# citibeth/spsparse

Measured on AMD Instinct MI355X. Metric: nnz(C)/s for C=A*A SpGEMM, higher is better.
Workload: dtype f64

## Files before the change

### spsparse_amd/csrc/consolidate.hip

```cpp
#include "internal.h"
#include "devutil.h"

namespace spsamd {

__global__ void k_inspect(const int32_t *major, const int32_t *minor, const double *val, size_t n,
	uint64_t nrow, uint64_t ncol, int zero_nan, uint32_t *flags)
{
	uint32_t f = 0;
	for (size_t i = (size_t)blockIdx.x * blockDim.x + threadIdx.x; i < n; i += (size_t)gridDim.x * blockDim.x) {
		int32_t r = major[i], c = minor[i];
		if (r < 0 || (uint64_t)r >= nrow || c < 0 || (uint64_t)c >= ncol) f |= 1u;
		double v = val[i];
		if (v == 0 || (zero_nan && v != v)) f |= 2u | 8u;
		if (i > 0) {
			int32_t pr = major[i - 1], pc = minor[i - 1];
			if (!(pr < r || (pr == r && pc < c))) f |= 2u;
			if (pr > r) f |= 16u;
			if (pr > r || (pr == r && pc > c)) f |= 32u;
			if (!(pc < c || (pc == c && pr < r))) f |= 4u;
		}
	}
	__shared__ uint32_t s_f;
	if (threadIdx.x == 0) s_f = 0;
	__syncthreads();
	uint32_t wf = 0;
#pragma unroll
	for (uint32_t b = 1u; b <= 32u; b <<= 1) if (__ballot(f & b)) wf |= b;
	if (wf && lane_id() == 0) atomicOr(&s_f, wf);
	__syncthreads();
	if (threadIdx.x == 0 && s_f && (*(volatile uint32_t *)flags & s_f) != s_f) atomicOr(flags, s_f);
}

__device__ __forceinline__ uint64_t ref_key(uint64_t key, int minor_bits, int major_bits, int swap)
{
	if (!swap) return key;
	const uint64_t minor = key & ((uint64_t(1) << minor_bits) - 1), major = key >> minor_bits;
	return (minor << major_bits) | major;
}

__global__ void k_gather_flag(const double *val, const uint32_t *perm, const uint64_t *keys, size_t n, int zero_nan,
	int minor_bits, int major_bits, int swap, double *sval, uint8_t *keep, unsigned long long *first_key)
{
	size_t i = (size_t)blockIdx.x * blockDim.x + threadIdx.x;
	if (i >= n) return;
	double v = val[perm[i]];
	sval[i] = v;
	keep[i] = (v != 0) ? 1 : 0;
	if (zero_nan && v != 0 && v == v) atomicMin(first_key, (unsigned long long)ref_key(keys[i], minor_bits, major_bits, swap));
}

__global__ void k_first_pos(const double *sval, const uint32_t *perm, const uint64_t *keys, size_t n,
	int minor_bits, int major_bits, int swap, const unsigned long long *first_key, uint32_t *first_pos)
{
	size_t i = (size_t)blockIdx.x * blockDim.x + threadIdx.x;
	if (i >= n) return;
	const double v = sval[i];
	if (v != 0 && v == v && ref_key(keys[i], minor_bits, major_bits, swap) == *first_key) atomicMin(first_pos, perm[i]);
}

__global__ void k_apply_first(const double *sval, const uint32_t *perm, const uint64_t *keys, uint8_t *keep, size_t n,
	int minor_bits, int major_bits, int swap, const unsigned long long *first_key, const uint32_t *first_pos)
{
	size_t i = (size_t)blockIdx.x * blockDim.x + threadIdx.x;
	if (i >= n) return;
	const double v = sval[i];
	if (v == v) return;
	const uint64_t k = ref_key(keys[i], minor_bits, major_bits, swap), fk = *first_key;
	if (k < fk || (k == fk && perm[i] < *first_pos)) keep[i] = 0;
}

__global__ void k_compact(const uint64_t *keys, const double *sval, const uint8_t *keep, const uint32_t *pos, size_t n,
	uint64_t *kk, double *kv)
{
	size_t i = (size_t)blockIdx.x * blockDim.x + threadIdx.x;
	if (i < n && keep[i]) {
		uint32_t p = pos[i];
		kk[p] = keys[i];
		kv[p] = sval[i];
	}
}

__global__ void k_heads(const uint64_t *kk, const uint32_t *nk_ptr, size_t n, uint8_t *head)
{
	size_t j = (size_t)blockIdx.x * blockDim.x + threadIdx.x;
	if (j >= n) return;
	uint32_t nk = *nk_ptr;
	head[j] = (j < nk && (j == 0 || kk[j] != kk[j - 1])) ? 1 : 0;
}

__global__ void k_merge(const uint64_t *kk, const double *kv, const uint8_t *head, const uint32_t *hpos,
	const uint32_t *nk_ptr, size_t n, int minor_bits, int policy,
	int32_t *row, int32_t *col, double *val)
{
	size_t j = (size_t)blockIdx.x * blockDim.x + threadIdx.x;
	if (j >= n || !head[j]) return;
	uint32_t nk = *nk_ptr;
	uint64_t key = kk[j];
	double acc = kv[j];
	for (size_t t = j + 1; t < nk && kk[t] == key; ++t) {
		if (policy == SPSAMD_ADD) acc += kv[t];
		else if (policy == SPSAMD_REPLACE) acc = kv[t];
	}
	uint32_t o = hpos[j];
	row[o] = (int32_t)(key >> minor_bits);
	col[o] = (int32_t)(key & ((uint64_t(1) << minor_bits) - 1));
	val[o] = acc;
}

__global__ void k_min_key(unsigned long long *first_key, const unsigned long long *global_key)
{
	if (*global_key < *first_key) *first_key = *global_key;
}

uint32_t inspect_operand(spsamd_ctx *c, const int32_t *major, const int32_t *minor, const double *val, size_t n,
	uint64_t nrow, uint64_t ncol)
{
	uint32_t *flags = c->arena.get<uint32_t>(1);
	fill_zero(c, flags, sizeof(uint32_t));
	if (n) {
		k_inspect<<<dim3(std::min(grid_for(n, 1024), 2048u)), dim3(256), 0, c->stream>>>(major, minor, val, n, nrow, ncol, 0, flags);
		SPS_LAUNCH_CHECK();
	}
	return read_back(c, flags);
}

void consolidate_operand(spsamd_ctx *c, const spsamd_coo *X, int lead, int ref_lead, int duplicate_policy, int zero_nan, ConMat *out,
	Prepared **prep, const unsigned long long *global_first_key)
{
	if (prep) *prep = nullptr;
// ... 21 lines not shown
	const int32_t *d1 = to_device(c, X->idx1, n, X->mem);
	const double *dv = to_device(c, X->val, n, X->mem);
	const int32_t *major = lead == 0 ? d0 : d1;
	const int32_t *minor = lead == 0 ? d1 : d0;

	uint32_t *flags = c->arena.get<uint32_t>(2);
	fill_zero(c, flags, 2 * sizeof(uint32_t));
	k_inspect<<<dim3(std::min(grid_for(n, 1024), 2048u)), dim3(256), 0, c->stream>>>(major, minor, dv, n, out->nrow, out->ncol, zero_nan, flags);
	SPS_LAUNCH_CHECK();
	uint32_t f = read_back(c, flags);
	if (f & 1u) throw Error{SPSAMD_EINVAL, "Sparse index out of bounds (VectorCooArray::add would reject it, VectorCooArray.hpp:246-262)"};

	if (X->sort0 == lead && (f & 16u))
		throw Error{SPSAMD_EINVAL, "operand claims sort_order but its leading index is not ascending (set_sorted() on unsorted tuples?)"};
	if ((X->sort0 == lead && !(zero_nan && ref_lead != lead && (f & 2u))) || !(f & 2u)) {
		out->row = const_cast<int32_t *>(major);
		out->col = const_cast<int32_t *>(minor);
		out->val = const_cast<double *>(dv);
		out->nnz = (uint32_t)n;
		return;
	}

	int mb = bits_of(out->ncol), Mb = bits_of(out->nrow);
	PairSort sort(c, n);
	build_keys(c, major, minor, n, mb, sort.keys);
	const int low_bit = (f & 4u) ? 0 : mb;
	sort.run(mb + Mb, low_bit);
	uint64_t *ks = sort.keys;
	uint32_t *ps = sort.perm;
	uint64_t *kk = sort.spare_keys;
	if (!(f & 4u) && !(f & 8u)) {
		out->row = c->arena.get<int32_t>(n);
		out->col = c->arena.get<int32_t>(n);
		out->val = c->arena.get<double>(n);
		gather_sorted(c, ks, ps, dv, n, mb, out->row, out->col, out->val);
		out->nnz = (uint32_t)n;
		return;
	}

	double *sval = c->arena.get<double>(n);
	uint8_t *keep = c->arena.get<uint8_t>(n);
	unsigned long long *first_key = c->arena.get<unsigned long long>(1);
	uint32_t *first_pos = flags + 1;
	const int swap = ref_lead != lead ? 1 : 0;
	if (zero_nan) {
		SPS_HIP(hipMemsetAsync(first_key, 0xFF, sizeof(unsigned long long), c->stream));
		fill_u32(c, first_pos, 0xFFFFFFFFu, 1);
	}
	k_gather_flag<<<dim3(grid_for(n)), dim3(256), 0, c->stream>>>(dv, ps, ks, n, zero_nan, mb, Mb, swap, sval, keep, first_key);
	SPS_LAUNCH_CHECK();
	if (zero_nan) {
		if (global_first_key) { k_min_key<<<dim3(1), dim3(1), 0, c->stream>>>(first_key, global_first_key); SPS_LAUNCH_CHECK(); }
		k_first_pos<<<dim3(grid_for(n)), dim3(256), 0, c->stream>>>(sval, ps, ks, n, mb, Mb, swap, first_key, first_pos);
		SPS_LAUNCH_CHECK();
		k_apply_first<<<dim3(grid_for(n)), dim3(256), 0, c->stream>>>(sval, ps, ks, keep, n, mb, Mb, swap, first_key, first_pos);
		SPS_LAUNCH_CHECK();
	}
	uint32_t *pos = c->arena.get<uint32_t>(n + 1);
	scan_exclusive_u8_u32(c, keep, pos, n);
	double *kv = c->arena.get<double>(n);
	k_compact<<<dim3(grid_for(n)), dim3(256), 0, c->stream>>>(ks, sval, keep, pos, n, kk, kv);
	SPS_LAUNCH_CHECK();
	uint8_t *head = keep;
	k_heads<<<dim3(grid_for(n)), dim3(256), 0, c->stream>>>(kk, pos + n, n, head);
	SPS_LAUNCH_CHECK();
	uint32_t *hpos = c->arena.get<uint32_t>(n + 1);
	scan_exclusive_u8_u32(c, head, hpos, n);
	out->row = c->arena.get<int32_t>(n);
	out->col = c->arena.get<int32_t>(n);
	out->val = c->arena.get<double>(n);
	k_merge<<<dim3(grid_for(n)), dim3(256), 0, c->stream>>>(kk, kv, head, hpos, pos + n, n, mb, duplicate_policy,
		out->row, out->col, out->val);
	SPS_LAUNCH_CHECK();
	out->nnz = read_back(c, hpos + n);
}

__global__ void k_first_key_raw(const int32_t *major, const int32_t *minor, const double *val, size_t n, int minor_bits, int major_bits, int swap,
	unsigned long long *first_key)
{
	unsigned long long best = ~0ull;
	for (size_t i = (size_t)blockIdx.x * blockDim.x + threadIdx.x; i < n; i += (size_t)gridDim.x * blockDim.x) {
		const double v = val[i];
		if (v != 0 && v == v) {
			const uint64_t key = ((uint64_t)(uint32_t)major[i] << minor_bits) | (uint64_t)(uint32_t)minor[i];
			const unsigned long long k = ref_key(key, minor_bits, major_bits, swap);
			best = k < best ? k : best;
		}
	}
#pragma unroll
	for (int d = 32; d >= 1; d >>= 1) { const unsigned long long o = __shfl_xor(best, d, 64); best = o < best ? o : best; }
	if (lane_id() == 0 && best != ~0ull) atomicMin(first_key, best);
}

void first_kept_key_raw(spsamd_ctx *c, const spsamd_coo *Xdev, int lead, int ref_lead, unsigned long long *out_dev)
{
	SPS_HIP(hipMemsetAsync(out_dev, 0xFF, sizeof(unsigned long long), c->stream));
	const size_t n = Xdev->nnz;
	if (!n) return;
	const uint64_t shape[2] = {Xdev->shape0, Xdev->shape1};
	const int mb = bits_of(shape[1 - lead]), Mb = bits_of(shape[lead]);
	const int32_t *major = lead == 0 ? Xdev->idx0 : Xdev->idx1, *minor = lead == 0 ? Xdev->idx1 : Xdev->idx0;
	k_first_key_raw<<<dim3(std::min(grid_for(n), 2048u)), dim3(256), 0, c->stream>>>(major, minor, Xdev->val, n, mb, Mb, ref_lead != lead ? 1 : 0, out_dev);
	SPS_LAUNCH_CHECK();
}

uint32_t *sorted_permutation(spsamd_ctx *c, const spsamd_coo *X, int lead)
{
	size_t n = X->nnz;
	if (n >= (size_t(1) << 31)) throw Error{SPSAMD_EINVAL, "operand has 2^31 or more tuples"};
	if (n == 0) return nullptr;
	if (!X->idx0 || !X->idx1) throw Error{SPSAMD_EINVAL, "operand with nnz > 0 has a null array"};
	uint64_t shape[2] = {X->shape0, X->shape1};
	const int32_t *d0 = to_device(c, X->idx0, n, X->mem);
	const int32_t *d1 = to_device(c, X->idx1, n, X->mem);
	const int32_t *major = lead == 0 ? d0 : d1;
	const int32_t *minor = lead == 0 ? d1 : d0;
	int mb = bits_of(shape[1 - lead]), Mb = bits_of(shape[lead]);
	PairSort sort(c, n);
	build_keys(c, major, minor, n, mb, sort.keys);
	sort.run(mb + Mb);
	return sort.perm;
}


__global__ void k_row_flags(const int32_t *row, size_t n, uint8_t *flag)
{
	size_t i = (size_t)blockIdx.x * blockDim.x + threadIdx.x;
	if (i < n) flag[i] = (i == 0 || row[i] != row[i - 1]) ? 1 : 0;
}

__global__ void k_row_starts(const int32_t *row, const uint8_t *flag, const uint32_t *pos, size_t n, uint32_t *beg, int32_t *id)
{
	size_t i = (size_t)blockIdx.x * blockDim.x + threadIdx.x;
	if (i >= n) return;
	if (flag[i]) {
		beg[pos[i]] = (uint32_t)i;
		id[pos[i]] = row[i];
	}
	if (i == n - 1) beg[pos[n]] = (uint32_t)n;
}

void dim_beginnings(spsamd_ctx *c, const ConMat &m, RowList *out)
{
	size_t n = m.nnz;
	out->nrows = 0;
	out->beg = c->arena.get<uint32_t>(n + 1);
	out->id = c->arena.get<int32_t>(n ? n : 1);
	if (n == 0) return;
	uint8_t *flag = c->arena.get<uint8_t>(n);
	uint32_t *pos = c->arena.get<uint32_t>(n + 1);
	k_row_flags<<<dim3(grid_for(n)), dim3(256), 0, c->stream>>>(m.row, n, flag);
	SPS_LAUNCH_CHECK();
	scan_exclusive_u8_u32(c, flag, pos, n);
	k_row_starts<<<dim3(grid_for(n)), dim3(256), 0, c->stream>>>(m.row, flag, pos, n, out->beg, out->id);
	SPS_LAUNCH_CHECK();
	out->nrows = read_back(c, pos + n);
}


__global__ void k_rowptr(const int32_t *row, uint32_t n, uint64_t nptr, uint32_t *ptr)
{
	uint64_t r = (uint64_t)blockIdx.x * blockDim.x + threadIdx.x;
	if (r >= nptr) return;
	uint32_t lo = 0, hi = n;
	while (lo < hi) {
		uint32_t mid = lo + ((hi - lo) >> 1);
		if ((uint64_t)(uint32_t)row[mid] < r) lo = mid + 1; else hi = mid;
	}
	ptr[r] = lo;
}

__global__ void k_rowptr_scatter(const int32_t *row, uint32_t n, uint64_t nptr, uint32_t *ptr)
{
	const uint64_t t = (uint64_t)blockIdx.x * blockDim.x + threadIdx.x;
	uint64_t first = 0, last = 0;
	if (t > 0 && t < n) {
		first = (uint64_t)(uint32_t)row[t - 1] + 1;
		last = std::min<uint64_t>((uint64_t)(uint32_t)row[t] + 1, nptr);
	}
// ... 69 lines not shown
```

### spsparse_amd/csrc/internal.h

```cpp
#pragma once

#include <hip/hip_runtime.h>
#include <stdint.h>
#include <stddef.h>
#include <string>
#include <vector>

#include "../../include/spsparse_amd.h"

namespace spsamd {


struct Error {
	int code;
	std::string msg;
};

#define SPS_HIP(call)                                                              \
	do {                                                                           \
		hipError_t e_ = (call);                                                    \
		if (e_ != hipSuccess)                                                      \
			throw ::spsamd::Error{SPSAMD_EHIP, std::string(#call) + ": " + hipGetErrorString(e_)}; \
	} while (0)

// ... 117 lines not shown
	EV_N3 = 6,
	EV_END = 7,
	EV_N4 = 8,
	EV_FETCH0 = EV_N4, EV_FETCH1 = 9 };
enum Ev2 { EV2_TILES_BEGIN = 0, EV2_TILES_END = 1, EV2_DIRECT_END = 2 };


void scan_exclusive_u32_i64(spsamd_ctx *c, const uint32_t *in, int64_t *out, size_t n);
void scan_exclusive_u32_u32(spsamd_ctx *c, const uint32_t *in, uint32_t *out, size_t n);
void scan_exclusive_u8_u32(spsamd_ctx *c, const uint8_t *in, uint32_t *out, size_t n);
void scan_exclusive_u64_u64(spsamd_ctx *c, const unsigned long long *in, unsigned long long *out, size_t n);

constexpr int SCAN_BATCH_MAX = 12;
struct ScanBatch { const uint32_t *in[SCAN_BATCH_MAX]; uint32_t *out[SCAN_BATCH_MAX]; int count = 0;
	void add(const uint32_t *i, uint32_t *o) { in[count] = i; out[count] = o; ++count; } };
void scan_exclusive_u32_batch(spsamd_ctx *c, const ScanBatch &b, size_t n);

constexpr int WORD_LIST_MAX = 40;
struct WordList { const uint32_t *p[WORD_LIST_MAX]; int count = 0;
	int add(const void *q) { p[count] = (const uint32_t *)q; return count++; }
	int add64(const void *q) { const int at = add(q); add((const uint32_t *)q + 1); return at; } };
void read_back_words(spsamd_ctx *c, const WordList &w, uint32_t *host);

struct PairSort {
	uint64_t *keys;
	uint32_t *perm;
	uint64_t *spare_keys;
	uint32_t *spare_pay;
	PairSort(spsamd_ctx *c, size_t n);
	void run(int key_bits, int low_bit = 0);
private:
	spsamd_ctx *c;
	size_t n;
};

void fill_u32(spsamd_ctx *c, uint32_t *p, uint32_t v, size_t n);
void fill_zero(spsamd_ctx *c, void *p, size_t bytes);
template <class T> T *get_zeroed(spsamd_ctx *c, size_t n) { T *p = c->arena.get<T>(n); fill_zero(c, p, n * sizeof(T)); return p; }

template <class T>
T read_back(spsamd_ctx *c, const T *dev)
{
	T *h = (T *)c->host_staging(sizeof(T));
	SPS_HIP(hipMemcpyAsync(h, dev, sizeof(T), hipMemcpyDeviceToHost, c->stream));
	SPS_HIP(hipStreamSynchronize(c->stream));
	return *h;
}

inline unsigned grid_for(size_t n, unsigned bs = 256) { return (unsigned)((n + bs - 1) / bs); }

#define SPSAMD_MEM_DEVICE_VERIFIED 3


struct Prepared;
// ... 14 lines not shown
	if (mem != SPSAMD_MEM_HOST || n == 0) return p;
	T *d = c->arena.get<T>(n);
	SPS_HIP(hipMemcpyAsync(d, p, n * sizeof(T), hipMemcpyHostToDevice, c->stream));
	return d;
}

struct PlainStream {
	const int32_t *major = nullptr, *minor = nullptr;
	const double *val = nullptr;
	uint32_t flags = 0;
	bool own_result = false;
};
PlainStream plain_stream(spsamd_ctx *c, const spsamd_coo &X, int lead);

struct MaskKeys {
	const int32_t *i = nullptr, *j = nullptr;
	uint32_t n = 0;
	Prepared *prep = nullptr;
};
void mask_keys(spsamd_ctx *c, const spsamd_coo *M, int lead, uint64_t nrow, uint64_t ncol, MaskKeys *out);

int bits_of(uint64_t dim);
void build_keys(spsamd_ctx *c, const int32_t *major, const int32_t *minor, size_t n, int minor_bits, uint64_t *keys);
void gather_sorted(spsamd_ctx *c, const uint64_t *keys, const uint32_t *perm, const double *val, size_t n, int minor_bits,
	int32_t *row, int32_t *col, double *oval);

struct ProductFrame {
	int a0, a1, bk, bj;
	uint64_t nrow, inner, ncol;
	uint64_t inner_b;
	uint64_t shape0, shape1;
	ProductFrame(const spsamd_coo *A, char transpose_A, const spsamd_coo *B, char transpose_B, bool permute);
	void check_inner(const char *what) const;
};
bool product_is_empty(double C, const spsamd_vec *scalei, const spsamd_coo *A, const spsamd_vec *scalej, const spsamd_coo *B,
	const spsamd_vec *scalek);


struct ConMat {
	int32_t *row = nullptr;
	int32_t *col = nullptr;
	double *val = nullptr;
	uint32_t nnz = 0;
	uint64_t nrow = 0, ncol = 0;
};


void consolidate_operand(spsamd_ctx *c, const spsamd_coo *X, int lead, int ref_lead, int duplicate_policy,
	int zero_nan, ConMat *out, Prepared **prep = nullptr, const unsigned long long *global_first_key = nullptr);

void first_kept_key_raw(spsamd_ctx *c, const spsamd_coo *Xdev, int lead, int ref_lead, unsigned long long *out_dev);

uint32_t inspect_operand(spsamd_ctx *c, const int32_t *major, const int32_t *minor, const double *val, size_t n,
	uint64_t nrow, uint64_t ncol);

struct RowList {
	uint32_t *beg = nullptr;
	int32_t *id = nullptr;
	uint32_t nrows = 0;
};
void dim_beginnings(spsamd_ctx *c, const ConMat &m, RowList *out);

uint32_t *sorted_permutation(spsamd_ctx *c, const spsamd_coo *X, int lead);

uint32_t *dense_rowptr(spsamd_ctx *c, const ConMat &m, uint32_t extra, uint32_t *into = nullptr);

struct __attribute__((packed, aligned(4))) BTup { int32_t col; uint32_t vlo, vhi; };

struct SolveSchedule {
	bool built = false;
	uint32_t levels = 0, max_level_rows = 0;
	uint64_t tuples_used = 0;
	int64_t zero_pivot = -1;
	uint32_t *level_ptr = nullptr;
	uint32_t *rows = nullptr;
	std::vector<uint32_t> h_level_ptr, h_level_max;
};

struct Prepared {
	spsamd_ctx *ctx = nullptr;
	ConMat m;
	int lead = 0;
	bool owns = false;
	std::vector<void *> owned;
// ... 141 lines not shown
```

### spsparse_amd/csrc/k_add.hip

```cpp
#include "internal.h"
#include "devutil.h"
#include "x86fp.h"

#include <algorithm>
#include <cstdio>
#include <cstring>

namespace spsamd {

struct FirstKept {
	unsigned long long key;
	uint32_t src, idx;
};

__device__ __forceinline__ uint64_t add_key(const int32_t *row, const int32_t *col, uint32_t i)
{
	return ((uint64_t)(uint32_t)row[i] << 32) | (uint64_t)(uint32_t)col[i];
}

__device__ __forceinline__ bool before_first(uint64_t key, uint32_t src, uint32_t idx, const FirstKept &f)
{
	return key < f.key || (key == f.key && (src < f.src || (src == f.src && idx < f.idx)));
}

// ... 161 lines not shown
}

static void add_stream(spsamd_ctx *c, const spsamd_coo *X, int lead, bool force_sort, AddStream *out, bool *sorted)
{
	*out = AddStream();
	const OperandView view = operand_view(c, X);
	if (view.prep && view.prep->lead == lead && !force_sort) { const ConMat &m = view.prep->m; out->row = m.row; out->col = m.col; out->val = m.val; out->n = m.nnz; return; }
	X = &view.coo;
	const size_t n = X->nnz;
	if (n == 0) return;
	const uint64_t shape[2] = {X->shape0, X->shape1};
	const PlainStream ps = plain_stream(c, *X, lead);
	const int32_t *major = ps.major, *minor = ps.minor;
	const double *dv = ps.val;
	const bool ordered = ps.own_result ? X->sort0 == lead : !(ps.flags & 32u);
	const int low_bit = !ps.own_result && !(ps.flags & 4u) ? -1 : 0;
	if (ordered && !force_sort) { out->row = major; out->col = minor; out->val = dv; out->n = (uint32_t)n; return; }
	const int mb = bits_of(shape[1 - lead]), Mb = bits_of(shape[lead]);
	PairSort sort(c, n);
	build_keys(c, major, minor, n, mb, sort.keys);
	sort.run(mb + Mb, low_bit < 0 ? mb : 0);
	int32_t *row = c->arena.get<int32_t>(n), *col = c->arena.get<int32_t>(n);
	double *val = c->arena.get<double>(n);
	gather_sorted(c, sort.keys, sort.perm, dv, n, mb, row, col, val);
	out->row = row; out->col = col; out->val = val; out->n = (uint32_t)n;
	*sorted = true;
}

template <int MODE>
static void launch_merge(spsamd_ctx *c, uint32_t ntiles, const AddStream &a, const AddStream &b, double alpha, double beta,
	int zero_nan, const FirstKept *first, const uint32_t *split, uint32_t *tile_count, const uint32_t *tile_off,
	int32_t *orow, int32_t *ocol, double *oval)
{
	k_add_merge<MODE><<<dim3(ntiles), dim3(ADD_NT), 0, c->stream>>>(a, b, alpha, beta, zero_nan, first, split, tile_count, tile_off, orow, ocol, oval);
	SPS_LAUNCH_CHECK();
}

void add_matrices(spsamd_ctx *c, double alpha, const spsamd_coo *A, char transpose_A, double beta, const spsamd_coo *B,
	char transpose_B, int duplicate_policy, int zero_nan, int sink_kind, int sink_flags, spsamd_result *res)
{
	check_sink_args(duplicate_policy, sink_kind);
	std::memset(res, 0, sizeof(*res));
	const int la = transpose_A == 'T' ? 1 : 0, lb = transpose_B == 'T' ? 1 : 0;
	const uint64_t ash[2] = {A->shape0, A->shape1}, bsh[2] = {B->shape0, B->shape1};
	const uint64_t nrow = ash[la], ncol = ash[1 - la];
	if (nrow != bsh[lb] || ncol != bsh[1 - lb]) {
		char buf[200];
// ... 55 lines not shown
```

### spsparse_amd/csrc/operand.hip

```cpp
#include "internal.h"
#include "devutil.h"

#include <algorithm>
#include <cstdio>

namespace spsamd {

OperandView operand_view(spsamd_ctx *c, const spsamd_coo *X)
{
	OperandView v;
	v.coo = *X;
	if (X->mem != SPSAMD_MEM_PREPARED) return v;
	Prepared *p = (Prepared *)const_cast<int32_t *>(X->idx0);
	if (!p || p->ctx != c) throw Error{SPSAMD_EINVAL, "a prepared operand belongs to the context that prepared it"};
	v.prep = p;
	v.coo.idx0 = p->lead == 0 ? p->m.row : p->m.col; v.coo.idx1 = p->lead == 0 ? p->m.col : p->m.row; v.coo.val = p->m.val;
	v.coo.nnz = p->m.nnz; v.coo.sort0 = p->lead; v.coo.mem = SPSAMD_MEM_DEVICE;
	return v;
}

uint64_t operand_tuples(const spsamd_coo *X)
{
	if (X->mem == SPSAMD_MEM_PREPARED) return X->idx0 ? ((const Prepared *)X->idx0)->m.nnz : 0;
	return X->nnz;
// ... 12 lines not shown
bool is_own_result(const spsamd_ctx *c, const spsamd_coo &X)
{
	if (X.mem != SPSAMD_MEM_DEVICE) return false;
	for (const auto &o : c->own)
		if (o.sort0 >= 0 && o.sort0 == X.sort0 && o.d0 == X.idx0 && o.d1 == X.idx1 && o.v == X.val && o.nnz == X.nnz &&
			o.shape0 == X.shape0 && o.shape1 == X.shape1) return true;
	return false;
}

int bits_of(uint64_t dim)
{
	int b = 0;
	while (b < 63 && (uint64_t(1) << b) < dim) ++b;
	return b;
}

__global__ void __launch_bounds__(256) k_build_keys(const int32_t *__restrict__ major, const int32_t *__restrict__ minor, uint32_t n,
	int minor_bits, uint64_t *__restrict__ keys)
{
	const uint32_t i = blockIdx.x * blockDim.x + threadIdx.x;
	if (i < n) keys[i] = ((uint64_t)(uint32_t)major[i] << minor_bits) | (uint64_t)(uint32_t)minor[i];
}

__global__ void __launch_bounds__(256) k_gather_sorted(const uint64_t *__restrict__ keys, const uint32_t *__restrict__ perm,
	const double *__restrict__ val, uint32_t n, int minor_bits, int32_t *__restrict__ row, int32_t *__restrict__ col,
	double *__restrict__ oval)
{
	const uint32_t i = blockIdx.x * blockDim.x + threadIdx.x;
	if (i >= n) return;
	const uint64_t k = keys[i];
	row[i] = (int32_t)(k >> minor_bits);
	col[i] = (int32_t)(k & ((uint64_t(1) << minor_bits) - 1));
	oval[i] = val[perm[i]];
}

void build_keys(spsamd_ctx *c, const int32_t *major, const int32_t *minor, size_t n, int minor_bits, uint64_t *keys)
{
	k_build_keys<<<dim3(grid_for(n)), dim3(256), 0, c->stream>>>(major, minor, (uint32_t)n, minor_bits, keys);
	SPS_LAUNCH_CHECK();
}

void gather_sorted(spsamd_ctx *c, const uint64_t *keys, const uint32_t *perm, const double *val, size_t n, int minor_bits,
	int32_t *row, int32_t *col, double *oval)
{
	k_gather_sorted<<<dim3(grid_for(n)), dim3(256), 0, c->stream>>>(keys, perm, val, (uint32_t)n, minor_bits, row, col, oval);
	SPS_LAUNCH_CHECK();
}

PlainStream plain_stream(spsamd_ctx *c, const spsamd_coo &X, int lead)
{
	check_operand(X, OPERAND_VALUES | OPERAND_PLAIN_MEM);
	const size_t n = X.nnz;
	const uint64_t shape[2] = {X.shape0, X.shape1};
	PlainStream s;
	s.own_result = is_own_result(c, X);
	const int32_t *d0 = to_device(c, X.idx0, n, X.mem), *d1 = to_device(c, X.idx1, n, X.mem);
	s.val = to_device(c, X.val, n, X.mem);
	s.major = lead == 0 ? d0 : d1; s.minor = lead == 0 ? d1 : d0;
	if (s.own_result) return s;
	s.flags = inspect_operand(c, s.major, s.minor, s.val, n, shape[lead], shape[1 - lead]);
	if (s.flags & 1u) throw Error{SPSAMD_EINVAL, "Sparse index out of bounds (VectorCooArray::add would reject it, VectorCooArray.hpp:246-262)"};
	if (X.sort0 == lead && (s.flags & 32u))
		throw Error{SPSAMD_EINVAL, "operand claims sort_order but its (row, col) keys are not in that order (set_sorted() on unsorted tuples?)"};
	return s;
}


__global__ void __launch_bounds__(256) k_mask_inspect(const int32_t *__restrict__ r, const int32_t *__restrict__ c, size_t n,
// ... 104 lines not shown
```

### spsparse_amd/csrc/prims.hip

```cpp
#include "internal.h"
#include "devutil.h"

#include <utility>

namespace spsamd {


static size_t round_up(size_t x, size_t a) { return (x + a - 1) / a * a; }

void *Arena::alloc(size_t bytes)
{
	bytes = round_up(bytes ? bytes : 1, 256);
	call_used += bytes;
	if (!slabs.empty()) {
		Slab &s = slabs.back();
		if (s.used + bytes <= s.cap) {
			void *p = s.p + s.used;
			s.used += bytes;
			return p;
		}
	}
	size_t cap = bytes > (size_t(256) << 20) ? bytes : (size_t(256) << 20);
	if (cap < high_water / 2) cap = high_water / 2;
	Slab s{nullptr, cap, 0};
// ... 302 lines not shown
{
	const int i = (int)threadIdx.x;
	if (i < w.count) dst[i] = *w.p[i];
}

void read_back_words(spsamd_ctx *c, const WordList &w, uint32_t *host)
{
	if (w.count == 0) return;
	uint32_t *dev = c->arena.get<uint32_t>(WORD_LIST_MAX);
	k_collect_words<<<dim3(1), dim3(64), 0, c->stream>>>(w, dev);
	SPS_LAUNCH_CHECK();
	uint32_t *h = (uint32_t *)c->host_staging(sizeof(uint32_t) * WORD_LIST_MAX);
	SPS_HIP(hipMemcpyAsync(h, dev, sizeof(uint32_t) * (size_t)w.count, hipMemcpyDeviceToHost, c->stream));
	SPS_HIP(hipStreamSynchronize(c->stream));
	for (int i = 0; i < w.count; ++i) host[i] = h[i];
}


constexpr int RS_NT = 256;
constexpr int RS_NW = RS_NT / 64;
constexpr int RS_ITER = 16;
constexpr int RS_TILE = RS_NT * RS_ITER;

template <int BITS>
__global__ __launch_bounds__(RS_NT) void k_rs_hist(const uint64_t *keys, size_t n, int shift, uint32_t *ghist, unsigned nblocks)
{
	constexpr int NB = 1 << BITS;
	__shared__ uint32_t hist[NB];
	for (int d = threadIdx.x; d < NB; d += RS_NT) hist[d] = 0;
	__syncthreads();
	size_t base = (size_t)blockIdx.x * RS_TILE;
#pragma unroll 4
	for (int q = 0; q < RS_ITER; ++q) {
		size_t i = base + (size_t)q * RS_NT + threadIdx.x;
		if (i < n) atomicAdd(&hist[(unsigned)(keys[i] >> shift) & (unsigned)(NB - 1)], 1u);
	}
	__syncthreads();
	for (int d = threadIdx.x; d < NB; d += RS_NT) ghist[(size_t)d * nblocks + blockIdx.x] = hist[d];
}

template <int BITS>
__global__ __launch_bounds__(RS_NT) void k_rs_scatter(const uint64_t *keys, const uint32_t *pay, size_t n, int shift,
	const uint32_t *gbase, unsigned nblocks, uint64_t *keys_out, uint32_t *pay_out, int iota_payload)
{
	constexpr int NB = 1 << BITS;
	constexpr int DPT = NB / RS_NT;
	__shared__ uint32_t wcnt[RS_NW][NB];
	__shared__ uint32_t gdelta[NB];
	__shared__ uint32_t scr[RS_NW + 1];
	__shared__ uint64_t s_key[RS_TILE];
	__shared__ uint32_t s_pay[RS_TILE];
	const unsigned w = wave_id(), lane = lane_id();
	for (int q = threadIdx.x; q < RS_NW * NB; q += RS_NT) (&wcnt[0][0])[q] = 0;
	__syncthreads();
	const size_t tile = (size_t)blockIdx.x * RS_TILE;
	const size_t wbase = tile + (size_t)w * (RS_ITER * 64);
	uint64_t key[RS_ITER];
#pragma unroll
	for (int q = 0; q < RS_ITER; ++q) {
		size_t i = wbase + (size_t)q * 64 + lane;
		key[q] = i < n ? keys[i] : 0;
		if (i < n) atomicAdd(&wcnt[w][(unsigned)(key[q] >> shift) & (unsigned)(NB - 1)], 1u);
	}
	__syncthreads();
	{
		uint32_t tot[DPT], mine = 0;
#pragma unroll
		for (int x = 0; x < DPT; ++x) {
			const unsigned d = threadIdx.x * DPT + x;
			tot[x] = 0;
#pragma unroll
			for (int ww = 0; ww < RS_NW; ++ww) tot[x] += wcnt[ww][d];
			mine += tot[x];
		}
		uint32_t lbase = block_exclusive_scan<uint32_t, RS_NT>(mine, scr, (uint32_t *)nullptr);
#pragma unroll
		for (int x = 0; x < DPT; ++x) {
			const unsigned d = threadIdx.x * DPT + x;
			gdelta[d] = gbase[(size_t)d * nblocks + blockIdx.x] - lbase;
			uint32_t run = lbase;
#pragma unroll
			for (int ww = 0; ww < RS_NW; ++ww) {
				uint32_t t = wcnt[ww][d];
				wcnt[ww][d] = run;
// ... 2 lines not shown
			lbase += tot[x];
		}
	}
	__syncthreads();
#pragma unroll
	for (int q = 0; q < RS_ITER; ++q) {
		size_t i = wbase + (size_t)q * 64 + lane;
		bool valid = i < n;
		unsigned digit = (unsigned)(key[q] >> shift) & (unsigned)(NB - 1);
		uint64_t peers = __ballot(valid);
#pragma unroll
		for (int b = 0; b < BITS; ++b) {
			bool bit = (digit >> b) & 1u;
			uint64_t m = __ballot(valid && bit);
			peers &= bit ? m : ~m;
		}
		unsigned rank = __popcll(peers & lanemask_lt());
		uint32_t old = 0;
		if (valid && rank == 0) old = atomicAdd(&wcnt[w][digit], (uint32_t)__popcll(peers));
		int leader = valid ? (__ffsll((unsigned long long)peers) - 1) : (int)lane;
		old = __shfl(old, leader, 64);
		if (valid) {
			s_key[old + rank] = key[q];
			s_pay[old + rank] = iota_payload ? (uint32_t)i : pay[i];
		}
	}
	__syncthreads();
	const uint32_t nvalid = (uint32_t)(n - tile < (size_t)RS_TILE ? n - tile : (size_t)RS_TILE);
	for (uint32_t p = threadIdx.x; p < nvalid; p += RS_NT) {
		const uint64_t k = s_key[p];
		const uint32_t dst = gdelta[(unsigned)(k >> shift) & (unsigned)(NB - 1)] + p;
		keys_out[dst] = k;
		pay_out[dst] = s_pay[p];
	}
}

template <int BITS>
static int radix_sort_pairs_bits(spsamd_ctx *c, uint64_t *keys0, uint32_t *pay0, uint64_t *keys1, uint32_t *pay1, size_t n, int key_bits, int low_bit)
{
	constexpr size_t NB = size_t(1) << BITS;
	int passes = (key_bits - low_bit + BITS - 1) / BITS;
	unsigned nblocks = (unsigned)((n + RS_TILE - 1) / RS_TILE);
	uint32_t *ghist = c->arena.get<uint32_t>(NB * nblocks);
	uint32_t *gbase = c->arena.get<uint32_t>(NB * nblocks + 1);
	uint64_t *ksrc = keys0, *kdst = keys1;
	uint32_t *psrc = pay0, *pdst = pay1;
	int where = 0;
	if (passes == 0) passes = 1;
	for (int p = 0; p < passes; ++p) {
		int shift = low_bit + BITS * p;
		k_rs_hist<BITS><<<dim3(nblocks), dim3(RS_NT), 0, c->stream>>>(ksrc, n, shift, ghist, nblocks);
		SPS_LAUNCH_CHECK();
		scan_exclusive_u32_u32(c, ghist, gbase, NB * nblocks);
		k_rs_scatter<BITS><<<dim3(nblocks), dim3(RS_NT), 0, c->stream>>>(ksrc, psrc, n, shift, gbase, nblocks, kdst, pdst, p == 0);
		SPS_LAUNCH_CHECK();
		uint64_t *tk = ksrc; ksrc = kdst; kdst = tk;
		uint32_t *tp = psrc; psrc = pdst; pdst = tp;
		where ^= 1;
	}
	return where;
}

static int radix_sort_pairs(spsamd_ctx *c, uint64_t *keys0, uint32_t *pay0, uint64_t *keys1, uint32_t *pay1, size_t n, int key_bits, int low_bit)
{
	if (n == 0) return 0;
	if (low_bit < 0 || low_bit > key_bits) low_bit = 0;
	return radix_sort_pairs_bits<8>(c, keys0, pay0, keys1, pay1, n, key_bits, low_bit);
}

PairSort::PairSort(spsamd_ctx *c, size_t n) : c(c), n(n)
{
	keys = c->arena.get<uint64_t>(n); spare_keys = c->arena.get<uint64_t>(n);
	perm = c->arena.get<uint32_t>(n); spare_pay = c->arena.get<uint32_t>(n);
}

void PairSort::run(int key_bits, int low_bit)
{
	if (radix_sort_pairs(c, keys, perm, spare_keys, spare_pay, n, key_bits, low_bit)) {
		std::swap(keys, spare_keys);
		std::swap(perm, spare_pay);
	}
}

}
```

### spsparse_amd/csrc/spgemm.hip

```cpp
#include "spgemm_host.h"

namespace spsamd {

__global__ void k_pack_b(const int32_t *bcol, const double *bval, uint32_t n, BTup *out)
{
	uint32_t i = blockIdx.x * blockDim.x + threadIdx.x;
	if (i >= n) return;
	double v = bval[i];
	BTup t; t.col = bcol[i]; t.vlo = (uint32_t)__double2loint(v); t.vhi = (uint32_t)__double2hiint(v);
	out[i] = t;
}


__global__ void k_elem_len(const int32_t *acol, const uint32_t *bptr, uint32_t n, uint32_t *lo, uint32_t *len)
{
	uint32_t e = blockIdx.x * blockDim.x + threadIdx.x;
	if (e < n) { int32_t k = acol[e]; uint32_t b = bptr[k]; lo[e] = b; len[e] = bptr[k + 1] - b; }
}

__global__ void k_apply_scalej(const int32_t *acol, const double *aval, uint32_t n, const int32_t *pos, const double *sval,
	int32_t ninner, int32_t *acol2, double *aval2)
{
	uint32_t e = blockIdx.x * blockDim.x + threadIdx.x;
	if (e >= n) return;
// ... 344 lines not shown
	Prepared *need[2]; int n = 0;
	if (!pa->have_maxlen) need[n++] = pa;
	if (pb != pa && !pb->have_maxlen) need[n++] = pb;
	if (!n) return;
	uint32_t *mx = get_zeroed<uint32_t>(c, 2);
	for (int q = 0; q < n; ++q) {
		k_max_rowlen<<<dim3(std::min(grid_for(need[q]->m.nrow, 1024), 1024u)), dim3(256), 0, st>>>(need[q]->rowptr, need[q]->m.nrow, mx + q);
		SPS_LAUNCH_CHECK();
	}
	struct { uint32_t a, b; } hm = read_back(c, (const decltype(hm) *)mx);
	need[0]->maxlen = hm.a; need[0]->have_maxlen = true;
	if (n > 1) { need[1]->maxlen = hm.b; need[1]->have_maxlen = true; }
}

void prepared_row_structure(spsamd_ctx *c, Prepared *p)
{
	ensure_rowptr(c, p);
	ensure_maxlen(c, p, p);
}

static const RowList &ensure_rowlist(spsamd_ctx *c, Prepared *p)
{
	if (p->have_rl) return p->rl;
	if (!p->owns) dim_beginnings(c, p->m, &p->rl);
	else {
		RowList tmp;
		dim_beginnings(c, p->m, &tmp);
		p->rl.nrows = tmp.nrows;
		p->rl.beg = p->get<uint32_t>((size_t)tmp.nrows + 1);
		p->rl.id = p->get<int32_t>(tmp.nrows ? tmp.nrows : 1);
		SPS_HIP(hipMemcpyAsync(p->rl.beg, tmp.beg, ((size_t)tmp.nrows + 1) * sizeof(uint32_t), hipMemcpyDeviceToDevice, c->stream));
		SPS_HIP(hipMemcpyAsync(p->rl.id, tmp.id, (size_t)tmp.nrows * sizeof(int32_t), hipMemcpyDeviceToDevice, c->stream));
	}
	p->have_rl = true;
	return p->rl;
}

static void wait_b_tuples(spsamd_ctx *c, MultiplyArgs &a)
{
	if (a.b_ready) { SPS_HIP(hipStreamWaitEvent(c->stream, a.b_ready, 0)); a.b_ready = nullptr; }
}

static BTup *ensure_btup(spsamd_ctx *c, MultiplyArgs &a, Prepared *p)
{
	if (p->btup) return p->btup;
	wait_b_tuples(c, a);
	p->btup = p->get<BTup>((size_t)p->m.nnz + DENSE_R);
	k_pack_b<<<dim3(grid_for(p->m.nnz)), dim3(256), 0, c->stream>>>(p->m.col, p->m.val, p->m.nnz, p->btup);
	SPS_LAUNCH_CHECK();
	return p->btup;
// ... 356 lines not shown
```

Baseline: 150.2 billion.

## Pack original index into sort key, fuse key build, merge runs in place

Packs the original element index into the low bits of the 64-bit radix-sort key when it fits. This drops the separate permutation payload arrays, and the first sort pass builds keys directly from the major/minor arrays instead of running a separate build_keys kernel. Consolidation replaces compact, heads and merge with a merge-runs pass over the sorted keys plus an emit pass, removing one scan and one compaction. Row beginnings are derived from an existing rowptr when available. In exchange, keys get wider, which can add radix passes, and threads walking long duplicate runs may diverge.

```diff
diff --git a/spsparse_amd/csrc/consolidate.hip b/spsparse_amd/csrc/consolidate.hip
--- a/spsparse_amd/csrc/consolidate.hip
+++ b/spsparse_amd/csrc/consolidate.hip
@@ -38,73 +38,76 @@
 	return (minor << major_bits) | major;
 }
 
-__global__ void k_gather_flag(const double *val, const uint32_t *perm, const uint64_t *keys, size_t n, int zero_nan,
+__global__ void k_gather_flag(const double *val, SortedKeys sk, size_t n, int zero_nan,
 	int minor_bits, int major_bits, int swap, double *sval, uint8_t *keep, unsigned long long *first_key)
 {
 	size_t i = (size_t)blockIdx.x * blockDim.x + threadIdx.x;
 	if (i >= n) return;
-	double v = val[perm[i]];
+	double v = val[sk.pos(i)];
 	sval[i] = v;
 	keep[i] = (v != 0) ? 1 : 0;
-	if (zero_nan && v != 0 && v == v) atomicMin(first_key, (unsigned long long)ref_key(keys[i], minor_bits, major_bits, swap));
-}
-
-__global__ void k_first_pos(const double *sval, const uint32_t *perm, const uint64_t *keys, size_t n,
+	if (zero_nan && v != 0 && v == v) atomicMin(first_key, (unsigned long long)ref_key(sk.key(i), minor_bits, major_bits, swap));
+}
+
+__global__ void k_first_pos(const double *sval, SortedKeys sk, size_t n,
 	int minor_bits, int major_bits, int swap, const unsigned long long *first_key, uint32_t *first_pos)
 {
 	size_t i = (size_t)blockIdx.x * blockDim.x + threadIdx.x;
 	if (i >= n) return;
 	const double v = sval[i];
-	if (v != 0 && v == v && ref_key(keys[i], minor_bits, major_bits, swap) == *first_key) atomicMin(first_pos, perm[i]);
-}
-
-__global__ void k_apply_first(const double *sval, const uint32_t *perm, const uint64_t *keys, uint8_t *keep, size_t n,
+	if (v != 0 && v == v && ref_key(sk.key(i), minor_bits, major_bits, swap) == *first_key) atomicMin(first_pos, sk.pos(i));
+}
+
+__global__ void k_apply_first(const double *sval, SortedKeys sk, uint8_t *keep, size_t n,
 	int minor_bits, int major_bits, int swap, const unsigned long long *first_key, const uint32_t *first_pos)
 {
 	size_t i = (size_t)blockIdx.x * blockDim.x + threadIdx.x;
 	if (i >= n) return;
 	const double v = sval[i];
 	if (v == v) return;
-	const uint64_t k = ref_key(keys[i], minor_bits, major_bits, swap), fk = *first_key;
-	if (k < fk || (k == fk && perm[i] < *first_pos)) keep[i] = 0;
-}
-
-__global__ void k_compact(const uint64_t *keys, const double *sval, const uint8_t *keep, const uint32_t *pos, size_t n,
-	uint64_t *kk, double *kv)
-{
-	size_t i = (size_t)blockIdx.x * blockDim.x + threadIdx.x;
-	if (i < n && keep[i]) {
-		uint32_t p = pos[i];
-		kk[p] = keys[i];
-		kv[p] = sval[i];
-	}
-}
-
-__global__ void k_heads(const uint64_t *kk, const uint32_t *nk_ptr, size_t n, uint8_t *head)
-{
-	size_t j = (size_t)blockIdx.x * blockDim.x + threadIdx.x;
-	if (j >= n) return;
-	uint32_t nk = *nk_ptr;
-	head[j] = (j < nk && (j == 0 || kk[j] != kk[j - 1])) ? 1 : 0;
-}
-
-__global__ void k_merge(const uint64_t *kk, const double *kv, const uint8_t *head, const uint32_t *hpos,
-	const uint32_t *nk_ptr, size_t n, int minor_bits, int policy,
+	const uint64_t k = ref_key(sk.key(i), minor_bits, major_bits, swap), fk = *first_key;
+	if (k < fk || (k == fk && sk.pos(i) < *first_pos)) keep[i] = 0;
+}
+
+template <class T> __device__ __forceinline__ void loaded(T &x) { asm volatile("" : "+v"(x)); }
+
+__global__ void k_merge_runs(SortedKeys sk, double *sval, const uint8_t *keep, size_t n, int policy, uint8_t *head)
+{
+	size_t i = (size_t)blockIdx.x * blockDim.x + threadIdx.x;
+	if (i >= n) return;
+	uint64_t key = sk.key(i), prev = sk.key(i ? i - 1 : 0), next = sk.key(i + 1 < n ? i + 1 : i);
+	uint32_t k0 = keep[i];
+	double acc = sval[i];
+	loaded(key); loaded(prev); loaded(next); loaded(k0); loaded(acc);
+	if (i > 0 && prev == key) { head[i] = 0; return; }
+	bool any = k0 != 0, moved = false;
+	for (size_t t = i + 1; t < n && next == key; ++t) {
+		uint32_t kt = keep[t];
+		double v = sval[t];
+		next = sk.key(t + 1 < n ? t + 1 : t);
+		loaded(kt); loaded(v); loaded(next);
+		if (!kt) continue;
+		if (!any) { acc = v; any = true; moved = true; }
+		else if (policy == SPSAMD_ADD) { acc += v; moved = true; }
+		else if (policy == SPSAMD_REPLACE) { acc = v; moved = true; }
+	}
+	head[i] = any ? 1 : 0;
+	if (moved) sval[i] = acc;
+}
+
+__global__ void k_emit_runs(SortedKeys sk, const double *sval, const uint8_t *head, const uint32_t *hpos, size_t n, int minor_bits,
 	int32_t *row, int32_t *col, double *val)
 {
-	size_t j = (size_t)blockIdx.x * blockDim.x + threadIdx.x;
-	if (j >= n || !head[j]) return;
-	uint32_t nk = *nk_ptr;
-	uint64_t key = kk[j];
-	double acc = kv[j];
-	for (size_t t = j + 1; t < nk && kk[t] == key; ++t) {
-		if (policy == SPSAMD_ADD) acc += kv[t];
-		else if (policy == SPSAMD_REPLACE) acc = kv[t];
-	}
-	uint32_t o = hpos[j];
+	size_t i = (size_t)blockIdx.x * blockDim.x + threadIdx.x;
+	if (i >= n) return;
+	uint32_t h = head[i], o = hpos[i];
+	uint64_t key = sk.key(i);
+	double v = sval[i];
+	loaded(h); loaded(o); loaded(key); loaded(v);
+	if (!h) return;
 	row[o] = (int32_t)(key >> minor_bits);
 	col[o] = (int32_t)(key & ((uint64_t(1) << minor_bits) - 1));
-	val[o] = acc;
+	val[o] = v;
 }
 
 __global__ void k_min_key(unsigned long long *first_key, const unsigned long long *global_key)
@@ -172,18 +175,15 @@
 	}
 
 	int mb = bits_of(out->ncol), Mb = bits_of(out->nrow);
-	PairSort sort(c, n);
-	build_keys(c, major, minor, n, mb, sort.keys);
+	PairSort sort(c, n, mb + Mb);
 	const int low_bit = (f & 4u) ? 0 : mb;
-	sort.run(mb + Mb, low_bit);
-	uint64_t *ks = sort.keys;
-	uint32_t *ps = sort.perm;
-	uint64_t *kk = sort.spare_keys;
+	sort.run_indices(major, minor, mb, mb + Mb, low_bit);
+	const SortedKeys sk = sort.sorted();
 	if (!(f & 4u) && !(f & 8u)) {
 		out->row = c->arena.get<int32_t>(n);
 		out->col = c->arena.get<int32_t>(n);
 		out->val = c->arena.get<double>(n);
-		gather_sorted(c, ks, ps, dv, n, mb, out->row, out->col, out->val);
+		gather_sorted(c, sk, dv, n, mb, out->row, out->col, out->val);
 		out->nnz = (uint32_t)n;
 		return;
 	}
@@ -197,30 +197,24 @@
 		SPS_HIP(hipMemsetAsync(first_key, 0xFF, sizeof(unsigned long long), c->stream));
 		fill_u32(c, first_pos, 0xFFFFFFFFu, 1);
 	}
-	k_gather_flag<<<dim3(grid_for(n)), dim3(256), 0, c->stream>>>(dv, ps, ks, n, zero_nan, mb, Mb, swap, sval, keep, first_key);
+	k_gather_flag<<<dim3(grid_for(n)), dim3(256), 0, c->stream>>>(dv, sk, n, zero_nan, mb, Mb, swap, sval, keep, first_key);
 	SPS_LAUNCH_CHECK();
 	if (zero_nan) {
 		if (global_first_key) { k_min_key<<<dim3(1), dim3(1), 0, c->stream>>>(first_key, global_first_key); SPS_LAUNCH_CHECK(); }
-		k_first_pos<<<dim3(grid_for(n)), dim3(256), 0, c->stream>>>(sval, ps, ks, n, mb, Mb, swap, first_key, first_pos);
+		k_first_pos<<<dim3(grid_for(n)), dim3(256), 0, c->stream>>>(sval, sk, n, mb, Mb, swap, first_key, first_pos);
 		SPS_LAUNCH_CHECK();
-		k_apply_first<<<dim3(grid_for(n)), dim3(256), 0, c->stream>>>(sval, ps, ks, keep, n, mb, Mb, swap, first_key, first_pos);
+		k_apply_first<<<dim3(grid_for(n)), dim3(256), 0, c->stream>>>(sval, sk, keep, n, mb, Mb, swap, first_key, first_pos);
 		SPS_LAUNCH_CHECK();
 	}
-	uint32_t *pos = c->arena.get<uint32_t>(n + 1);
-	scan_exclusive_u8_u32(c, keep, pos, n);
-	double *kv = c->arena.get<double>(n);
-	k_compact<<<dim3(grid_for(n)), dim3(256), 0, c->stream>>>(ks, sval, keep, pos, n, kk, kv);
-	SPS_LAUNCH_CHECK();
-	uint8_t *head = keep;
-	k_heads<<<dim3(grid_for(n)), dim3(256), 0, c->stream>>>(kk, pos + n, n, head);
+	uint8_t *head = c->arena.get<uint8_t>(n);
+	k_merge_runs<<<dim3(grid_for(n)), dim3(256), 0, c->stream>>>(sk, sval, keep, n, duplicate_policy, head);
 	SPS_LAUNCH_CHECK();
 	uint32_t *hpos = c->arena.get<uint32_t>(n + 1);
 	scan_exclusive_u8_u32(c, head, hpos, n);
 	out->row = c->arena.get<int32_t>(n);
 	out->col = c->arena.get<int32_t>(n);
 	out->val = c->arena.get<double>(n);
-	k_merge<<<dim3(grid_for(n)), dim3(256), 0, c->stream>>>(kk, kv, head, hpos, pos + n, n, mb, duplicate_policy,
-		out->row, out->col, out->val);
+	k_emit_runs<<<dim3(grid_for(n)), dim3(256), 0, c->stream>>>(sk, sval, head, hpos, n, mb, out->row, out->col, out->val);
 	SPS_LAUNCH_CHECK();
 	out->nnz = read_back(c, hpos + n);
 }
@@ -252,6 +246,12 @@
 	const int32_t *major = lead == 0 ? Xdev->idx0 : Xdev->idx1, *minor = lead == 0 ? Xdev->idx1 : Xdev->idx0;
 	k_first_key_raw<<<dim3(std::min(grid_for(n), 2048u)), dim3(256), 0, c->stream>>>(major, minor, Xdev->val, n, mb, Mb, ref_lead != lead ? 1 : 0, out_dev);
 	SPS_LAUNCH_CHECK();
+}
+
+__global__ void k_word_pos(SortedKeys sk, size_t n, uint32_t *perm)
+{
+	size_t i = (size_t)blockIdx.x * blockDim.x + threadIdx.x;
+	if (i < n) perm[i] = sk.pos(i);
 }
 
 uint32_t *sorted_permutation(spsamd_ctx *c, const spsamd_coo *X, int lead)
@@ -266,10 +266,13 @@
 	const int32_t *major = lead == 0 ? d0 : d1;
 	const int32_t *minor = lead == 0 ? d1 : d0;
 	int mb = bits_of(shape[1 - lead]), Mb = bits_of(shape[lead]);
-	PairSort sort(c, n);
-	build_keys(c, major, minor, n, mb, sort.keys);
-	sort.run(mb + Mb);
-	return sort.perm;
+	PairSort sort(c, n, mb + Mb);
+	sort.run_indices(major, minor, mb, mb + Mb);
+	if (sort.perm) return sort.perm;
+	uint32_t *perm = c->arena.get<uint32_t>(n);
+	k_word_pos<<<dim3(grid_for(n)), dim3(256), 0, c->stream>>>(sort.sorted(), n, perm);
+	SPS_LAUNCH_CHECK();
+	return perm;
 }
 
 
@@ -305,6 +308,40 @@
 	k_row_starts<<<dim3(grid_for(n)), dim3(256), 0, c->stream>>>(m.row, flag, pos, n, out->beg, out->id);
 	SPS_LAUNCH_CHECK();
 	out->nrows = read_back(c, pos + n);
+}
+
+__global__ void k_ptr_flags(const uint32_t *ptr, uint64_t nrow, uint8_t *flag)
+{
+	uint64_t r = (uint64_t)blockIdx.x * blockDim.x + threadIdx.x;
+	if (r < nrow) flag[r] = ptr[r + 1] > ptr[r] ? 1 : 0;
+}
+
+__global__ void k_ptr_starts(const uint32_t *ptr, const uint8_t *flag, const uint32_t *pos, uint64_t nrow, uint32_t *beg, int32_t *id)
+{
+	uint64_t r = (uint64_t)blockIdx.x * blockDim.x + threadIdx.x;
+	if (r >= nrow) return;
+	if (flag[r]) {
+		beg[pos[r]] = ptr[r];
+		id[pos[r]] = (int32_t)r;
+	}
+	if (r == nrow - 1) beg[pos[nrow]] = ptr[nrow];
+}
+
+void dim_beginnings(spsamd_ctx *c, const ConMat &m, const uint32_t *ptr, RowList *out)
+{
+	const uint64_t nrow = m.nrow;
+	out->nrows = 0;
+	out->beg = c->arena.get<uint32_t>(nrow + 1);
+	out->id = c->arena.get<int32_t>(nrow ? nrow : 1);
+	if (m.nnz == 0) return;
+	uint8_t *flag = c->arena.get<uint8_t>(nrow);
+	uint32_t *pos = c->arena.get<uint32_t>(nrow + 1);
+	k_ptr_flags<<<dim3(grid_for(nrow)), dim3(256), 0, c->stream>>>(ptr, nrow, flag);
+	SPS_LAUNCH_CHECK();
+	scan_exclusive_u8_u32(c, flag, pos, nrow);
+	k_ptr_starts<<<dim3(grid_for(nrow)), dim3(256), 0, c->stream>>>(ptr, flag, pos, nrow, out->beg, out->id);
+	SPS_LAUNCH_CHECK();
+	out->nrows = read_back(c, pos + nrow);
 }
 
 
diff --git a/spsparse_amd/csrc/internal.h b/spsparse_amd/csrc/internal.h
--- a/spsparse_amd/csrc/internal.h
+++ b/spsparse_amd/csrc/internal.h
@@ -163,14 +163,26 @@
 	int add64(const void *q) { const int at = add(q); add((const uint32_t *)q + 1); return at; } };
 void read_back_words(spsamd_ctx *c, const WordList &w, uint32_t *host);
 
+struct SortedKeys {
+	const uint64_t *w;
+	const uint32_t *perm;
+	int ibits;
+	__device__ __forceinline__ uint64_t key(size_t i) const { return w[i] >> ibits; }
+	__device__ __forceinline__ uint32_t pos(size_t i) const { return perm ? perm[i] : (uint32_t)(w[i] & ((uint64_t(1) << ibits) - 1)); }
+};
+
 struct PairSort {
 	uint64_t *keys;
 	uint32_t *perm;
+	int index_bits;
+	PairSort(spsamd_ctx *c, size_t n, int word_key_bits = -1);
+	void run(int key_bits, int low_bit = 0);
+	void run_indices(const int32_t *major, const int32_t *minor, int minor_bits, int key_bits, int low_bit = 0);
+	SortedKeys sorted() const { return SortedKeys{keys, perm, index_bits < 0 ? 0 : index_bits}; }
+private:
 	uint64_t *spare_keys;
 	uint32_t *spare_pay;
-	PairSort(spsamd_ctx *c, size_t n);
-	void run(int key_bits, int low_bit = 0);
-private:
+	void sort_from(const void *first, int key_bits, int low_bit);
 	spsamd_ctx *c;
 	size_t n;
 };
@@ -231,7 +243,7 @@
 
 int bits_of(uint64_t dim);
 void build_keys(spsamd_ctx *c, const int32_t *major, const int32_t *minor, size_t n, int minor_bits, uint64_t *keys);
-void gather_sorted(spsamd_ctx *c, const uint64_t *keys, const uint32_t *perm, const double *val, size_t n, int minor_bits,
+void gather_sorted(spsamd_ctx *c, const SortedKeys &sk, const double *val, size_t n, int minor_bits,
 	int32_t *row, int32_t *col, double *oval);
 
 struct ProductFrame {
@@ -269,6 +281,7 @@
 	uint32_t nrows = 0;
 };
 void dim_beginnings(spsamd_ctx *c, const ConMat &m, RowList *out);
+void dim_beginnings(spsamd_ctx *c, const ConMat &m, const uint32_t *ptr, RowList *out);
 
 uint32_t *sorted_permutation(spsamd_ctx *c, const spsamd_coo *X, int lead);
 
diff --git a/spsparse_amd/csrc/k_add.hip b/spsparse_amd/csrc/k_add.hip
--- a/spsparse_amd/csrc/k_add.hip
+++ b/spsparse_amd/csrc/k_add.hip
@@ -207,7 +207,7 @@
 	sort.run(mb + Mb, low_bit < 0 ? mb : 0);
 	int32_t *row = c->arena.get<int32_t>(n), *col = c->arena.get<int32_t>(n);
 	double *val = c->arena.get<double>(n);
-	gather_sorted(c, sort.keys, sort.perm, dv, n, mb, row, col, val);
+	gather_sorted(c, sort.sorted(), dv, n, mb, row, col, val);
 	out->row = row; out->col = col; out->val = val; out->n = (uint32_t)n;
 	*sorted = true;
 }
diff --git a/spsparse_amd/csrc/operand.hip b/spsparse_amd/csrc/operand.hip
--- a/spsparse_amd/csrc/operand.hip
+++ b/spsparse_amd/csrc/operand.hip
@@ -58,16 +58,17 @@
 	if (i < n) keys[i] = ((uint64_t)(uint32_t)major[i] << minor_bits) | (uint64_t)(uint32_t)minor[i];
 }
 
-__global__ void __launch_bounds__(256) k_gather_sorted(const uint64_t *__restrict__ keys, const uint32_t *__restrict__ perm,
+__global__ void __launch_bounds__(256) k_gather_sorted(SortedKeys sk,
 	const double *__restrict__ val, uint32_t n, int minor_bits, int32_t *__restrict__ row, int32_t *__restrict__ col,
 	double *__restrict__ oval)
 {
 	const uint32_t i = blockIdx.x * blockDim.x + threadIdx.x;
 	if (i >= n) return;
-	const uint64_t k = keys[i];
+	const uint64_t k = sk.key(i);
+	const double v = val[sk.pos(i)];
 	row[i] = (int32_t)(k >> minor_bits);
 	col[i] = (int32_t)(k & ((uint64_t(1) << minor_bits) - 1));
-	oval[i] = val[perm[i]];
+	oval[i] = v;
 }
 
 void build_keys(spsamd_ctx *c, const int32_t *major, const int32_t *minor, size_t n, int minor_bits, uint64_t *keys)
@@ -76,10 +77,10 @@
 	SPS_LAUNCH_CHECK();
 }
 
-void gather_sorted(spsamd_ctx *c, const uint64_t *keys, const uint32_t *perm, const double *val, size_t n, int minor_bits,
+void gather_sorted(spsamd_ctx *c, const SortedKeys &sk, const double *val, size_t n, int minor_bits,
 	int32_t *row, int32_t *col, double *oval)
 {
-	k_gather_sorted<<<dim3(grid_for(n)), dim3(256), 0, c->stream>>>(keys, perm, val, (uint32_t)n, minor_bits, row, col, oval);
+	k_gather_sorted<<<dim3(grid_for(n)), dim3(256), 0, c->stream>>>(sk, val, (uint32_t)n, minor_bits, row, col, oval);
 	SPS_LAUNCH_CHECK();
 }
 
diff --git a/spsparse_amd/csrc/prims.hip b/spsparse_amd/csrc/prims.hip
--- a/spsparse_amd/csrc/prims.hip
+++ b/spsparse_amd/csrc/prims.hip
@@ -348,8 +348,20 @@
 constexpr int RS_ITER = 16;
 constexpr int RS_TILE = RS_NT * RS_ITER;
 
+struct KeySrc {
+	const uint64_t *keys;
+	const int32_t *major, *minor;
+	int minor_bits, index_bits;
+	__device__ __forceinline__ uint64_t at(size_t i) const
+	{
+		if (keys) return keys[i];
+		const uint64_t k = ((uint64_t)(uint32_t)major[i] << minor_bits) | (uint64_t)(uint32_t)minor[i];
+		return index_bits < 0 ? k : (k << index_bits) | i;
+	}
+};
+
 template <int BITS>
-__global__ __launch_bounds__(RS_NT) void k_rs_hist(const uint64_t *keys, size_t n, int shift, uint32_t *ghist, unsigned nblocks)
+__global__ __launch_bounds__(RS_NT) void k_rs_hist(KeySrc keys, size_t n, int shift, uint32_t *ghist, unsigned nblocks)
 {
 	constexpr int NB = 1 << BITS;
 	__shared__ uint32_t hist[NB];
@@ -359,14 +371,14 @@
 #pragma unroll 4
 	for (int q = 0; q < RS_ITER; ++q) {
 		size_t i = base + (size_t)q * RS_NT + threadIdx.x;
-		if (i < n) atomicAdd(&hist[(unsigned)(keys[i] >> shift) & (unsigned)(NB - 1)], 1u);
+		if (i < n) atomicAdd(&hist[(unsigned)(keys.at(i) >> shift) & (unsigned)(NB - 1)], 1u);
 	}
 	__syncthreads();
 	for (int d = threadIdx.x; d < NB; d += RS_NT) ghist[(size_t)d * nblocks + blockIdx.x] = hist[d];
 }
 
-template <int BITS>
-__global__ __launch_bounds__(RS_NT) void k_rs_scatter(const uint64_t *keys, const uint32_t *pay, size_t n, int shift,
+template <int BITS, bool PAY>
+__global__ __launch_bounds__(RS_NT) void k_rs_scatter(KeySrc keys, const uint32_t *pay, size_t n, int shift,
 	const uint32_t *gbase, unsigned nblocks, uint64_t *keys_out, uint32_t *pay_out, int iota_payload)
 {
 	constexpr int NB = 1 << BITS;
@@ -375,7 +387,7 @@
 	__shared__ uint32_t gdelta[NB];
 	__shared__ uint32_t scr[RS_NW + 1];
 	__shared__ uint64_t s_key[RS_TILE];
-	__shared__ uint32_t s_pay[RS_TILE];
+	__shared__ uint32_t s_pay[PAY ? RS_TILE : 1];
 	const unsigned w = wave_id(), lane = lane_id();
 	for (int q = threadIdx.x; q < RS_NW * NB; q += RS_NT) (&wcnt[0][0])[q] = 0;
 	__syncthreads();
@@ -385,7 +397,7 @@
 #pragma unroll
 	for (int q = 0; q < RS_ITER; ++q) {
 		size_t i = wbase + (size_t)q * 64 + lane;
-		key[q] = i < n ? keys[i] : 0;
+		key[q] = i < n ? keys.at(i) : 0;
 		if (i < n) atomicAdd(&wcnt[w][(unsigned)(key[q] >> shift) & (unsigned)(NB - 1)], 1u);
 	}
 	__syncthreads();
@@ -434,7 +446,7 @@
 		old = __shfl(old, leader, 64);
 		if (valid) {
 			s_key[old + rank] = key[q];
-			s_pay[old + rank] = iota_payload ? (uint32_t)i : pay[i];
+			if constexpr (PAY) s_pay[old + rank] = iota_payload ? (uint32_t)i : pay[i];
 		}
 	}
 	__syncthreads();
@@ -443,12 +455,12 @@
 		const uint64_t k = s_key[p];
 		const uint32_t dst = gdelta[(unsigned)(k >> shift) & (unsigned)(NB - 1)] + p;
 		keys_out[dst] = k;
-		pay_out[dst] = s_pay[p];
+		if constexpr (PAY) pay_out[dst] = s_pay[p];
 	}
 }
 
 template <int BITS>
-static int radix_sort_pairs_bits(spsamd_ctx *c, uint64_t *keys0, uint32_t *pay0, uint64_t *keys1, uint32_t *pay1, size_t n, int key_bits, int low_bit)
+static int radix_sort_pairs_bits(spsamd_ctx *c, const KeySrc *first, uint64_t *keys0, uint32_t *pay0, uint64_t *keys1, uint32_t *pay1, size_t n, int key_bits, int low_bit)
 {
 	constexpr size_t NB = size_t(1) << BITS;
 	int passes = (key_bits - low_bit + BITS - 1) / BITS;
@@ -461,10 +473,12 @@
 	if (passes == 0) passes = 1;
 	for (int p = 0; p < passes; ++p) {
 		int shift = low_bit + BITS * p;
-		k_rs_hist<BITS><<<dim3(nblocks), dim3(RS_NT), 0, c->stream>>>(ksrc, n, shift, ghist, nblocks);
+		const KeySrc src = p == 0 && first ? *first : KeySrc{ksrc, nullptr, nullptr, 0, -1};
+		k_rs_hist<BITS><<<dim3(nblocks), dim3(RS_NT), 0, c->stream>>>(src, n, shift, ghist, nblocks);
 		SPS_LAUNCH_CHECK();
 		scan_exclusive_u32_u32(c, ghist, gbase, NB * nblocks);
-		k_rs_scatter<BITS><<<dim3(nblocks), dim3(RS_NT), 0, c->stream>>>(ksrc, psrc, n, shift, gbase, nblocks, kdst, pdst, p == 0);
+		if (pay0) k_rs_scatter<BITS, true><<<dim3(nblocks), dim3(RS_NT), 0, c->stream>>>(src, psrc, n, shift, gbase, nblocks, kdst, pdst, p == 0);
+		else k_rs_scatter<BITS, false><<<dim3(nblocks), dim3(RS_NT), 0, c->stream>>>(src, nullptr, n, shift, gbase, nblocks, kdst, nullptr, 0);
 		SPS_LAUNCH_CHECK();
 		uint64_t *tk = ksrc; ksrc = kdst; kdst = tk;
 		uint32_t *tp = psrc; psrc = pdst; pdst = tp;
@@ -473,25 +487,38 @@
 	return where;
 }
 
-static int radix_sort_pairs(spsamd_ctx *c, uint64_t *keys0, uint32_t *pay0, uint64_t *keys1, uint32_t *pay1, size_t n, int key_bits, int low_bit)
+static int radix_sort_pairs(spsamd_ctx *c, const KeySrc *first, uint64_t *keys0, uint32_t *pay0, uint64_t *keys1, uint32_t *pay1, size_t n, int key_bits, int low_bit)
 {
 	if (n == 0) return 0;
 	if (low_bit < 0 || low_bit > key_bits) low_bit = 0;
-	return radix_sort_pairs_bits<8>(c, keys0, pay0, keys1, pay1, n, key_bits, low_bit);
-}
-
-PairSort::PairSort(spsamd_ctx *c, size_t n) : c(c), n(n)
-{
+	return radix_sort_pairs_bits<8>(c, first, keys0, pay0, keys1, pay1, n, key_bits, low_bit);
+}
+
+PairSort::PairSort(spsamd_ctx *c, size_t n, int word_key_bits) : c(c), n(n)
+{
+	const int ib = bits_of(n);
+	index_bits = word_key_bits >= 0 && word_key_bits + ib <= 64 ? ib : -1;
 	keys = c->arena.get<uint64_t>(n); spare_keys = c->arena.get<uint64_t>(n);
-	perm = c->arena.get<uint32_t>(n); spare_pay = c->arena.get<uint32_t>(n);
-}
-
-void PairSort::run(int key_bits, int low_bit)
-{
-	if (radix_sort_pairs(c, keys, perm, spare_keys, spare_pay, n, key_bits, low_bit)) {
+	perm = spare_pay = nullptr;
+	if (index_bits < 0) { perm = c->arena.get<uint32_t>(n); spare_pay = c->arena.get<uint32_t>(n); }
+}
+
+void PairSort::sort_from(const void *first, int key_bits, int low_bit)
+{
+	const int up = index_bits < 0 ? 0 : index_bits;
+	if (low_bit < 0 || low_bit > key_bits) low_bit = 0;
+	if (radix_sort_pairs(c, (const KeySrc *)first, keys, perm, spare_keys, spare_pay, n, key_bits + up, low_bit + up)) {
 		std::swap(keys, spare_keys);
 		std::swap(perm, spare_pay);
 	}
 }
 
-}
+void PairSort::run(int key_bits, int low_bit) { sort_from(nullptr, key_bits, low_bit); }
+
+void PairSort::run_indices(const int32_t *major, const int32_t *minor, int minor_bits, int key_bits, int low_bit)
+{
+	const KeySrc src{nullptr, major, minor, minor_bits, index_bits};
+	sort_from(&src, key_bits, low_bit);
+}
+
+}
diff --git a/spsparse_amd/csrc/spgemm.hip b/spsparse_amd/csrc/spgemm.hip
--- a/spsparse_amd/csrc/spgemm.hip
+++ b/spsparse_amd/csrc/spgemm.hip
@@ -390,10 +390,12 @@
 static const RowList &ensure_rowlist(spsamd_ctx *c, Prepared *p)
 {
 	if (p->have_rl) return p->rl;
-	if (!p->owns) dim_beginnings(c, p->m, &p->rl);
+	const bool by_ptr = p->rowptr && p->m.nrow + 1 <= (uint64_t)p->m.nnz;
+	auto beginnings = [&](RowList *out) { if (by_ptr) dim_beginnings(c, p->m, p->rowptr, out); else dim_beginnings(c, p->m, out); };
+	if (!p->owns) beginnings(&p->rl);
 	else {
 		RowList tmp;
-		dim_beginnings(c, p->m, &tmp);
+		beginnings(&tmp);
 		p->rl.nrows = tmp.nrows;
 		p->rl.beg = p->get<uint32_t>((size_t)tmp.nrows + 1);
 		p->rl.id = p->get<int32_t>(tmp.nrows ? tmp.nrows : 1);
```

Result: faster. 152.8 billion, median of 6 (+1.7%).
